# YuePanEdward/GH-ICP

Hardware: AMD Instinct MI355X
Metric: registered_pairs_per_sec (higher is better)
Workload: dtype f64

## Files before the change

gh-icp_amd/api.py:

```python
from __future__ import annotations

import ctypes as C
import os

import numpy as np

_HERE = os.path.dirname(os.path.abspath(__file__))
LIB_PATH = os.environ.get("GHICP_LIB") or os.path.join(_HERE, "libghicp_hip.so")

FEATURE_BSC, FEATURE_ROPS, FEATURE_FPFH, FEATURE_NONE = 0, 1, 2, 3
CORR_NN, CORR_NNR, CORR_KM = 0, 1, 2


class Params(C.Structure):
    _fields_ = [("feature", C.c_int32), ("corr", C.c_int32), ("dof", C.c_int32), ("max_iter", C.c_int32),
                ("radius_nonmax", C.c_float), ("adjust_ratio", C.c_float), ("adjust_step", C.c_float),
                ("est_iou", C.c_float), ("converge_t", C.c_float), ("converge_r", C.c_float),
                ("bbx_magnitude", C.c_float), ("pad_", C.c_float),
                ("penalty_initial", C.c_double), ("para1", C.c_double), ("para2", C.c_double),
                ("km_eps", C.c_double), ("min_cor", C.c_int32), ("weight_changing_rate", C.c_int32)]


class Iter(C.Structure):
    _fields_ = [("cor", C.c_int32), ("converged", C.c_int32)] + [
# ... 169 lines not shown
            raise GhicpError("ghicp error %d: %s" % (rc, self.lib.ghicp_last_error(self.h).decode()))

    def sync(self):
        self._check(self.lib.ghicp_ctx_synchronize(self.h))

    def kernel_timing(self, on=True):
        self._check(self.lib.ghicp_ctx_kernel_timing(self.h, 1 if on else 0))

    def km_launch_stats(self):
        out = (C.c_double * 8)()
        self._check(self.lib.ghicp_ctx_km_launch_stats(self.h, out))
        keys = ("launches", "solves", "mean_solve_ms", "mean_longest_solve_ms", "mean_launch_span_ms", "slots", "idle_slot_fraction", "worst_longest_over_mean")
        return dict(zip(keys, (float(v) for v in out)))

    def pair_loop_stats(self):
        out = (C.c_double * 8)()
        self._check(self.lib.ghicp_ctx_pair_loop_stats(self.h, out))
        keys = ("launches", "slots", "solves", "mean_solve_ms", "longest_solve_ms", "mean_launch_span_ms", "idle_slot_fraction", "solve_share_of_slot_time")
        return dict(zip(keys, (float(v) for v in out)))

    def loop_progress(self):
        a, t = C.c_int64(0), C.c_int64(0)
        self.lib.ghicp_ctx_loop_progress(self.h, C.byref(a), C.byref(t))
        return a.value, t.value

    def loop_progress_reset(self, total):
        self._check(self.lib.ghicp_ctx_loop_progress_reset(self.h, C.c_int64(int(total))))

    def set_loop_cost_hints(self, cost):
        c = np.ascontiguousarray(cost, dtype=np.float32)
        self._check(self.lib.ghicp_ctx_set_loop_cost_hints(self.h, C.c_int32(c.size), c.ctypes.data_as(C.POINTER(C.c_float))))

    def loop_timeline(self, detail=False):
# ... 501 lines not shown
```

gh-icp_amd/csrc/ctx.h:

```cpp
#pragma once
#include <hip/hip_runtime.h>

#include <atomic>
#include <cstdarg>
#include <cstdio>
#include <cstring>
#include <string>
#include <vector>

#include "../../include/ghicp_c.h"

#define GH_HIP(call)                                                                                          \
  do {                                                                                                        \
    hipError_t e_ = (call);                                                                                   \
    if (e_ != hipSuccess) return ctx->fail(GHICP_ERR_HIP, "%s:%d %s -> %s", __FILE__, __LINE__, #call, hipGetErrorString(e_)); \
  } while (0)
#define GH_TRY(call)               \
  do {                             \
    int r_ = (call);               \
    if (r_ != GHICP_OK) return r_; \
  } while (0)
#define GH_ARG(cond)                                                                \
  do {                                                                              \
    if (!(cond)) return ctx->fail(GHICP_ERR_ARG, "%s: bad argument (%s)", __func__, #cond); \
// ... 23 lines not shown
  }
  template <typename T> T* as() const { return reinterpret_cast<T*>(p); }
  void release() { if (p) (void)hipFree(p); p = nullptr; cap = 0; }
};

enum BufSlot {
  B_STAGE0 = 0, B_STAGE1, B_STAGE2, B_STAGE3, B_STAGE4, B_STAGE5, B_STAGE6, B_STAGE7,
  B_LOOP_STATE, B_LOOP_KPS, B_LOOP_PARTMIN, B_LOOP_PARTIDX, B_LOOP_PARTSUM, B_LOOP_PARTMIN2, B_LOOP_PARTIDX2, B_LOOP_FDT,
  B_LOOP_SP, B_LOOP_TP, B_LOOP_TRACE, B_LOOP_WFD, B_LOOP_KMW, B_LOOP_KMMATCH, B_LOOP_KMSCR, B_LOOP_ACC,
  B_GRID_KEYS, B_GRID_KEYS2, B_GRID_VALS, B_GRID_VALS2, B_GRID_TMP, B_GRID_START, B_GRID_PTS, B_GRID_MISC,
  B_GRID2_KEYS, B_GRID2_KEYS2, B_GRID2_VALS, B_GRID2_VALS2, B_GRID2_START, B_GRID2_PTS,
  B_FE_LAMBDA, B_FE_CURV, B_FE_COUNT, B_FE_CAND, B_FE_STATE, B_FE_KP, B_FE_SORTK, B_FE_SORTK2, B_FE_SORTV, B_FE_SORTV2, B_FE_CPTS,
  B_FE_FLAGS, B_FE_SCAN, B_FE_SCATTER,
  B_P_KEEP_S, B_P_KEEP_T, B_P_DS_S, B_P_DS_T, B_P_KP_S, B_P_KP_T, B_P_KPXYZ_S, B_P_KPXYZ_T, B_P_FEAT_S, B_P_FEAT_T, B_P_LCS,
  B_P_FD, B_P_MISC, B_P_PATTERN, B_FD_JOBS, B_TRANSFORM_JOBS,
  B_KM_LX, B_KM_MISC, B_KM_SLACK, B_KM_LSTAT, B_KM_ORDER,
  B_FB_DESC, B_FB_HEADPOS, B_FB_DS, B_FB_ORD,
  B_PRIM_TMP, B_NMSR_KEY, B_NMSR_CELL, B_NMSR_TABLE, B_NMSR_HEAD, B_NMSR_PTS, B_NMSR_SKEY, B_NMSR_STATE, B_NMSR_NEXT, B_NMSR_SEL, B_NMSR_MISC, B_NMSR_LIST, B_NMSR_PTS0, B_NMSR_SKEY0,
  B_ICP_TC_KEYS, B_ICP_TC_KEYS2, B_ICP_TC_VALS, B_ICP_TC_VALS2, B_ICP_TC_START, B_ICP_TC_PTS,
  B_ICP_SC_KEYS, B_ICP_SC_KEYS2, B_ICP_SC_VALS, B_ICP_SC_VALS2, B_ICP_SC_START, B_ICP_SC_PTS,
  B_ICP_CUR, B_ICP_Q, B_ICP_NN, B_ICP_ND, B_ICP_NN2, B_ICP_ND2, B_ICP_KEYS, B_ICP_KEYS2, B_ICP_SORTTMP, B_ICP_PART, B_ICP_STATE,
  B_ICP_PEND, B_ICP_TNRM, B_ICP_OUT,
  B_GICP_COVS, B_GICP_COVT, B_GICP_MAHAL, B_GICP_SRC4,
  B_NUM
};

enum KtSlot { KT_PCA = 0, KT_BSC, KT_KM_SOLVE, KT_CD_ROWMIN, KT_KM_WEIGHTS, KT_FD_BSC, KT_NMS_ROUND, KT_VOXEL_SORT,
              KT_FB_VOXEL, KT_FB_GRID, KT_FB_PRUNE, KT_FB_RANK, KT_FB_OUT,
              KT_PAIR_LOOP,
              KT_TRANSFORM,
              KT_PAIR_LOOP_DISPATCH,
// ... 27 lines not shown
    if (!kt_on || !a) return;
    hipEvent_t b = kt_event();
    (void)hipEventRecord(b, st);
    kt_pending.push_back({slot, a, b});
  }
  void kt_collect() {
    for (auto& p : kt_pending) {
      float ms = 0;
      if (hipEventElapsedTime(&ms, p.a, p.b) == hipSuccess) { kt_ms[p.slot] += ms; kt_count[p.slot]++; }
      kt_pool.push_back(p.a);
      kt_pool.push_back(p.b);
    }
    kt_pending.clear();
  }
  static constexpr int KM_LSTAT_MAX = 8192;
  static constexpr int KM_LSTAT_W = 8;
  long long km_launches = 0;
  std::vector<int> km_slots;
  long long loop_hazards = 0;
  std::vector<float> loop_cost_hints;
  std::vector<long long> loop_timeline;
  std::atomic<long long> loop_active{0}, loop_total{0};
  bool bbox_valid = false;
  const float* bbox_ptr = nullptr;
  long long bbox_n = 0;
  int bbox_stride = 0;
  float bbox_mm[6] = {0, 0, 0, 0, 0, 0};
  int device = 0;
  hipStream_t stream = nullptr;
  hipStream_t own_stream = nullptr;
  bool km_stats = false, km_force_hazard = false;
  int loop_slots_cap = 0;
  bool loop_confine = true;
  double loop_confine_margin = 1.15;
  hipStream_t confine_stream = nullptr, rest_stream = nullptr;
  int confine_cus = 0;
  struct ConfinePair { int cus; hipStream_t confined, rest; };
  std::vector<ConfinePair> confine_cache;
  bool km_compact = true;
  int km_compact_from = 0;
  int km_kflags() const { return (km_force_hazard ? 4 : 0) | (km_compact_from << 8); }
  int loop_min_lds = 0;
  std::vector<uint32_t> cu_mask;
  std::vector<hipStream_t> aux_streams;
  std::vector<hipEvent_t> aux_events;
  int* progress_host = nullptr;
  std::atomic<bool> progress_live{false};
  bool host_ptrs = false;
  struct Staged { const void* host; size_t bytes; uint64_t fp; void* dev; uint64_t tick; };
  std::vector<Staged> staged;
  size_t staged_bytes = 0;
  uint64_t stage_tick = 0;
  long long staged_hits = 0, staged_misses = 0;
  void stage_clear() {
    if (staged.empty()) return;
    (void)hipStreamSynchronize(stream);
// ... 180 lines not shown
```

gh-icp_amd/csrc/ctx.hip:

```cpp
#include "ctx.h"
#include "devmath.h"

extern "C" const char* ghicp_version(void) { return "ghicp-hip 0.1 (gfx950)"; }

extern "C" void ghicp_params_default(ghicp_params* p) {
  if (!p) return;
  memset(p, 0, sizeof(*p));
  p->feature = GHICP_FEATURE_BSC;
  p->corr = GHICP_CORR_KM;
  p->dof = 6;
  p->max_iter = 200;
  p->radius_nonmax = 1.5f;
  p->adjust_ratio = 1.1f;
  p->adjust_step = 0.1f;
  p->est_iou = 0.6f;
  p->converge_t = 0.02f;
  p->converge_r = 0.02f;
  p->bbx_magnitude = 0.f;
  p->penalty_initial = 2.0;
  p->para1 = 1.0;
  p->para2 = 1.0;
  p->km_eps = 0.01;
  p->min_cor = 10;
  p->weight_changing_rate = 6;
// ... 3 lines not shown
  if (!out) return GHICP_ERR_ARG;
  *out = nullptr;
  int count = 0;
  if (hipGetDeviceCount(&count) != hipSuccess || count <= 0 || device < 0 || device >= count) return GHICP_ERR_NO_GPU;
  if (hipSetDevice(device) != hipSuccess) return GHICP_ERR_NO_GPU;
  hipDeviceProp_t prop;
  if (hipGetDeviceProperties(&prop, device) != hipSuccess) return GHICP_ERR_NO_GPU;
  ghicp_ctx* c = new ghicp_ctx();
  c->device = device;
  c->num_cu = prop.multiProcessorCount > 0 ? prop.multiProcessorCount : 256;
  c->km_stats = getenv("GHICP_KM_STATS") != nullptr;
  c->km_force_hazard = getenv("GHICP_KM_FORCE_HAZARD") != nullptr;
  if (const char* e = getenv("GHICP_LOOP_SLOTS")) c->loop_slots_cap = atoi(e) > 0 ? atoi(e) : 0;
  if (const char* e = getenv("GHICP_LOOP_CONFINE")) c->loop_confine = atoi(e) != 0;
  if (const char* e = getenv("GHICP_KM_COMPACT")) c->km_compact = atoi(e) != 0;
  if (const char* e = getenv("GHICP_KM_COMPACT_FROM")) c->km_compact_from = atoi(e) > 0 && atoi(e) < 65535 ? atoi(e) : 0;
  if (const char* e = getenv("GHICP_LOOP_MIN_LDS")) c->loop_min_lds = atoi(e) > 0 ? atoi(e) : 0;
  if (const char* e = getenv("GHICP_LOOP_CONFINE_MARGIN")) { const double m = atof(e); if (m >= 0.25 && m <= 4.0) c->loop_confine_margin = m; }
  if (hipHostMalloc(&c->pinned, 4096, hipHostMallocDefault) != hipSuccess) { delete c; return GHICP_ERR_HIP; }
  c->pinned_cap = 4096;
  *out = c;
  return GHICP_OK;
}

extern "C" int ghicp_ctx_destroy(ghicp_ctx* ctx) {
  if (!ctx) return GHICP_OK;
  (void)hipSetDevice(ctx->device);
  (void)hipDeviceSynchronize();
  ctx->kt_collect();
  for (hipEvent_t e : ctx->kt_pool) (void)hipEventDestroy(e);
// ... 398 lines not shown
```

gh-icp_amd/csrc/km4.hip:

```cpp
#include "km4_dev.h"

#include <algorithm>
#include <vector>
#include <cstdlib>

namespace {

template <bool PROF, bool CP>
__global__ __launch_bounds__(K4_T, CP ? 4 : 1) void k_km4(const Km2Problem* __restrict__ probs, int flags, int lds_bytes, unsigned long long* __restrict__ lstat,
                                                        const int* __restrict__ order, unsigned short* __restrict__ scr, long long scr_stride) {
  const Km2Problem P = probs[order ? order[blockIdx.x] : (int)blockIdx.x];
  if (P.n <= 0 || (P.done && *P.done)) return;
  if (k4_takes_compact(P.n, flags, lds_bytes) != CP) return;
  extern __shared__ __attribute__((aligned(16))) char smem[];
  k4_solve_block<PROF, CP>(P, flags, smem, lds_bytes, lstat, CP && scr ? (k4_gu16)(scr + (size_t)blockIdx.x * (size_t)scr_stride) : (k4_gu16) nullptr);
}

}

size_t gh_km4_lds_bytes_compact(int n) { return (size_t)k4_lds_need(n, true) + 16; }

size_t gh_km4_slot_bytes(int n, bool compact_on) {
  const size_t quarter = 160 * 1024 / 4, std_b = gh_km4_lds_bytes(n);
  return (compact_on && std_b > quarter && gh_km4_lds_bytes_compact(n) <= quarter) ? gh_km4_lds_bytes_compact(n) : std_b;
// ... 129 lines not shown
    worst = std::max(worst, (double)r[3] / ((double)r[2] / (double)r[4]));
  }
  if (used == 0) return GHICP_OK;
  out8[0] = (double)used; out8[1] = solves; out8[2] = sum_dt / solves * tick_ms; out8[3] = sum_max / (double)used * tick_ms;
  out8[4] = sum_span / (double)used * tick_ms; out8[5] = slots; out8[6] = cap > 0 ? 1.0 - sum_dt / cap : 0.0; out8[7] = worst;
  return GHICP_OK;
}

extern "C" int ghicp_ctx_loop_hazards(ghicp_ctx* ctx, int64_t* solves) {
  GH_ENTER(ctx);
  GH_ARG(solves != nullptr);
  *solves = (int64_t)ctx->loop_hazards;
  return GHICP_OK;
}

extern "C" int ghicp_ctx_pair_loop_stats(ghicp_ctx* ctx, double* out8) {
  GH_ENTER(ctx);
  GH_ARG(out8 != nullptr);
  for (int i = 0; i < 8; i++) out8[i] = 0.0;
  const long long nl = ctx->km_launches;
  if (nl <= 0 || !ctx->buf[B_KM_LSTAT].p) return GHICP_OK;
  for (hipStream_t a : ctx->aux_streams) GH_HIP(hipStreamSynchronize(a));
  GH_HIP(hipStreamSynchronize(ctx->stream));
  constexpr int W = ghicp_ctx::KM_LSTAT_W;
  std::vector<unsigned long long> h((size_t)nl * W);
  GH_HIP(hipMemcpy(h.data(), ctx->buf[B_KM_LSTAT].p, h.size() * sizeof(unsigned long long), hipMemcpyDeviceToHost));
  const double tick_ms = 1e3 / 100e6;
  double launches = 0, slots = 0, solves = 0, sum_dt = 0, mx = 0, sum_span = 0, life = 0, cap = 0;
  for (long long l = 0; l < nl; l++) {
    const unsigned long long* r = &h[(size_t)l * W];
    if (r[6] == 0) continue;
    const double start = (double)((1ull << 62) - r[0]), span = (double)r[1] - start;
    launches++; slots += (double)r[6]; solves += (double)r[4]; sum_dt += (double)r[2]; mx = std::max(mx, (double)r[3]);
    sum_span += span; life += (double)r[5]; cap += std::min((double)ctx->km_slots[(size_t)l], (double)r[6]) * span;
  }
  if (launches == 0) return GHICP_OK;
  out8[0] = launches; out8[1] = slots; out8[2] = solves; out8[3] = solves > 0 ? sum_dt / solves * tick_ms : 0.0; out8[4] = mx * tick_ms;
  out8[5] = sum_span / launches * tick_ms; out8[6] = cap > 0 ? 1.0 - life / cap : 0.0; out8[7] = life > 0 ? sum_dt / life : 0.0;
  return GHICP_OK;
}
```

gh-icp_amd/csrc/loop.hip:

```cpp
#include "ctx.h"
#include "devmath.h"

#include <cmath>

#include "km_prob.h"
#include "km4_dev.h"
int gh_km_solve_dev(ghicp_ctx* ctx, const double* w, int n, double eps, int32_t* match, const int* done_flag);

namespace {

struct LoopState {
  int it, done, cor, converged_flag;
  double RMS, FDM, FDstd, IoU, para1, para2, penalty, CDmean, CDstd, energy;
  double Rt_till[16];
  double rmse_after;
  unsigned long long t_begin, t_end;
  unsigned long long t_solve_max;
  int it_solve_max;
  unsigned hw_id;
};

struct LoopConst {
  int ks, kt, n, feature, corr, max_iter, min_cor, nchunk_a, nchunk_b, chunk_a, chunk_b, nparts;
  float scale, est_iou, adjust_ratio, adjust_step;
// ... 79 lines not shown
    if (threadIdx.x == 0) {
      const size_t b = (size_t)by * cdiv_dev(ka, ROWS) + bx;
      P.psum[b * 2] = bs;
      P.psum[b * 2 + 1] = bs2;
    }
  }
}

template <int FT, bool COLS>
__global__ __launch_bounds__(ROWS) void k_cd_rowmin(const LoopProb* __restrict__ probs) {
  const LoopProb& P = probs[blockIdx.z];
  if (P.st->done) return;
  __shared__ double sB[CHUNK_MAX * 3];
  __shared__ double red[16];
  dev_cd_rowmin<FT, COLS>(P, (int)blockIdx.x, (int)blockIdx.y, sB, red);
}

__device__ inline void dev_penalty(const LoopProb& P, double* red) {
  LoopState* st = P.st;
  const LoopConst& C = P.C;
  double s = 0, s2 = 0;
  for (int i = threadIdx.x; i < C.nparts; i += blockDim.x) { s += P.psum[i * 2]; s2 += P.psum[i * 2 + 1]; }
  s = gh_block_sum(s, red);
  s2 = gh_block_sum(s2, red);
  if (threadIdx.x == 0) {
    const int it = st->it;
    const double cnt = (double)C.ks * (double)C.kt;
    double piv, wfd0 = 0, wed0 = 1;
    if (C.feature == GHICP_FEATURE_BSC) { wfd0 = P.wfd[it]; wed0 = 1.0 - wfd0; }
    const double inv_k0 = 1.0 / (double)(it + 1);
    if (C.feature == GHICP_FEATURE_BSC) piv = cd_pivot<GHICP_FEATURE_BSC>(P, wed0, wfd0, inv_k0);
    else if (C.feature == GHICP_FEATURE_FPFH) piv = cd_pivot<GHICP_FEATURE_FPFH>(P, wed0, wfd0, inv_k0);
    else piv = cd_pivot<GHICP_FEATURE_NONE>(P, wed0, wfd0, inv_k0);
    const double dm = s / (double)C.kt / (double)C.ks;
    const double mean = piv + dm;
    double var = s2 / cnt - dm * dm;
    if (var < 0) var = 0;
    const double sd = sqrt(var);
    double pen;
    if (C.feature == GHICP_FEATURE_NONE) {
      pen = fmax(mean, 1.0);
      st->CDstd = 0;
    } else if (C.feature == GHICP_FEATURE_BSC) {
      const double wfd = P.wfd[it], wed = 1.0 - wfd;
      if (it > 1) pen = st->RMS * st->para1 * (double)C.scale * wed + (st->FDM + st->para2 * st->FDstd) * wfd;
      else pen = mean - C.penalty_initial * sd;
      pen = fmax(pen, 5.0);
      st->CDstd = sd;
    } else {
      if (it > 1) pen = st->RMS * st->para1 * (double)C.scale * st->para2;
      else pen = mean / C.penalty_initial;
      st->CDstd = 0;
    }
    st->CDmean = mean;
    st->penalty = pen;
  }
}

__global__ __launch_bounds__(256) void k_penalty(const LoopProb* __restrict__ probs) {
  const LoopProb& P = probs[blockIdx.x];
  if (P.st->done) return;
  __shared__ double red[16];
  dev_penalty(P, red);
}

// ... 356 lines not shown
    }
  __syncthreads();
  dev_penalty(P, red);
  __syncthreads();
}
template <int FT>
__device__ __noinline__ void pl_graph(const LoopProb& P, int* ired) {
  const int rb4 = cdiv_dev(P.C.n, 4);
  for (int bx = 0; bx < rb4; bx++) dev_km_csr<FT, 0>(P, bx);
  __syncthreads();
  dev_km_scan_desc(P, ired);
  __syncthreads();
  for (int bx = 0; bx < rb4; bx++) dev_km_csr<FT, 1>(P, bx);
  __syncthreads();
}
template <bool PROF>
__device__ __noinline__ void pl_km(const Km2Problem* desc, int km_flags, char* smem, int lds_bytes) {
  const Km2Problem KP = *desc;
  k4_solve_block<PROF, false>(KP, km_flags, smem, lds_bytes, nullptr, (k4_gu16) nullptr);
  __syncthreads();
}
template <bool PROF>
__device__ __noinline__ void pl_km_compact(const Km2Problem* desc, int km_flags, char* smem, int lds_bytes, k4_gu16 scr) {
  const Km2Problem KP = *desc;
  k4_solve_block<PROF, true>(KP, km_flags, smem, lds_bytes, nullptr, scr);
  __syncthreads();
}
template <int FT>
__device__ __noinline__ void pl_solve(const LoopProb& P, double* red, int* ired, double* sh) {
  dev_solve<FT>(P, red, ired, sh);
  __syncthreads();
}

template <int FT, bool PROF>
__global__ __launch_bounds__(K4_T, 4) void k_pair_loop(const LoopProb* __restrict__ probs, const int* __restrict__ order, const int npairs, int* qhead,
                                                  const int km_flags, const int lds_bytes, unsigned long long* lstat, int* progress,
                                                  const int* __restrict__ order2, const int npairs2, int* qhead2,
                                                  unsigned short* __restrict__ scr, const long long scr_stride) {
  extern __shared__ __attribute__((aligned(16))) char smem[];
  double* sB = reinterpret_cast<double*>(smem);
  double* red = sB + CHUNK_MAX * 3;
  double* sh = red + 16;
  int* ired = reinterpret_cast<int*>(sh + 32);
  volatile int* s_idx = ired + 18;
  const unsigned long long t_slot0 = lstat ? __builtin_amdgcn_s_memrealtime() : 0ull;
  unsigned long long t_solve = 0ull, t_solve_max = 0ull, n_solve = 0ull;
  __builtin_amdgcn_s_setprio(3);
  for (int qsel = 0; qsel < 2; qsel++) {
  const int* const ord = qsel == 0 ? order : order2;
  const int np = qsel == 0 ? npairs : npairs2;
  int* const qh = qsel == 0 ? qhead : qhead2;
  if (ord == nullptr) break;
  for (;;) {
    __syncthreads();
    if (threadIdx.x == 0) *s_idx = atomicAdd(qh, 1);
    __syncthreads();
    const int q = *s_idx;
    if (q >= np) break;
    const LoopProb& P = probs[ord[q]];
    if (threadIdx.x == 0 && lstat) P.st->t_begin = __builtin_amdgcn_s_memrealtime();
    unsigned long long t_pair_max = 0ull;
    int it_pair_max = 0;
    while (*(volatile int*)&P.st->done == 0) {
      pl_sweep<FT>(P, sB, red);
      pl_graph<FT>(P, ired);
      const unsigned long long t0 = lstat ? __builtin_amdgcn_s_memrealtime() : 0ull;
      if (k4_takes_compact(P.C.n, km_flags, lds_bytes))
        pl_km_compact<PROF>(P.km_desc, km_flags, smem, lds_bytes, scr ? (k4_gu16)(scr + (size_t)blockIdx.x * (size_t)scr_stride) : (k4_gu16) nullptr);
      else
        pl_km<PROF>(P.km_desc, km_flags, smem, lds_bytes);
      if (lstat) {
        const unsigned long long dt = __builtin_amdgcn_s_memrealtime() - t0;
        t_solve += dt; t_solve_max = dt > t_solve_max ? dt : t_solve_max; n_solve++;
        if (dt > t_pair_max) { t_pair_max = dt; it_pair_max = *(volatile int*)&P.st->it; }
      }
      pl_solve<FT>(P, red, ired, sh);
    }
    if (threadIdx.x == 0 && lstat) {
      P.st->t_end = __builtin_amdgcn_s_memrealtime();
      P.st->t_solve_max = t_pair_max;
      P.st->it_solve_max = it_pair_max;
      P.st->hw_id = ((unsigned)__builtin_amdgcn_s_getreg((4) | (0 << 6) | (31 << 11)) & 0xFFFFu) | (((unsigned)__builtin_amdgcn_s_getreg((20) | (0 << 6) | (3 << 11)) & 0xFu) << 16);
    }
    if (threadIdx.x == 0 && progress) __hip_atomic_fetch_add(progress, 1, __ATOMIC_RELAXED, __HIP_MEMORY_SCOPE_SYSTEM);
  }
  }
  if (threadIdx.x == 0 && lstat) {
    const unsigned long long t1 = __builtin_amdgcn_s_memrealtime();
    atomicMax(&lstat[0], (1ull << 62) - t_slot0);
    atomicMax(&lstat[1], t1);
    atomicAdd(&lstat[2], t_solve);
    atomicMax(&lstat[3], t_solve_max);
    atomicAdd(&lstat[4], n_solve);
    atomicAdd(&lstat[5], t1 - t_slot0);
    atomicAdd(&lstat[6], 1ull);
  }
}

static void pick_chunks(int ka, int kb, int batch, int* chunk, int* nchunk) {
  const int rowblocks = cdiv(ka > 0 ? ka : 1, ROWS) * (batch > 0 ? batch : 1);
  int want = cdiv(2048, rowblocks);
  int ch = cdiv(kb > 0 ? kb : 1, want);
  if (ch < 32) ch = 32;
  if (ch > CHUNK_MAX) ch = CHUNK_MAX;
  *chunk = ch;
  *nchunk = kb > 0 ? cdiv(kb, ch) : 1;
}

struct Carver {
  char* base;
// ... 49 lines not shown
  size_t scr_next = 0;
  {
    int n_all = 1;
    bool need = ctx->km_compact_from > 0;
    for (int c = 0; c < nc; c++) {
      n_all = std::max(n_all, plan.nmax[c]);
      const size_t lds = std::max(std::max(plan.lds[c], (size_t)PL_SCRATCH + 64), (size_t)ctx->loop_min_lds);
      need = need || k4_lds_need(plan.nmax[c], false) > (long long)lds;
    }
    if (need) {
      scr_stride = k4_scratch_u16(n_all);
      size_t slots = 0;
      for (int c = 0; c < nc; c++) slots += 2 * (size_t)std::min(plan.count[c], 4 * ctx->num_cu);
      GH_TRY(ctx->reserve(B_KM_SLACK, slots * (size_t)scr_stride, &scr));
    }
  }
  GH_HIP(hipMemsetAsync(dqheads, 0, 16 * sizeof(int), s));
  unsigned long long* lstat = nullptr;
  int batch_slots = 0, batch_grid = 0;
  if (ctx->kt_on && ctx->km_launches < ghicp_ctx::KM_LSTAT_MAX) {
    GH_TRY(ctx->reserve(B_KM_LSTAT, (size_t)ghicp_ctx::KM_LSTAT_MAX * ghicp_ctx::KM_LSTAT_W, &lstat));
    lstat += ctx->km_launches * ghicp_ctx::KM_LSTAT_W;
  }
  int confine_b = 0;
  if (ctx->loop_confine && nc == 2 && plan.per_cu[0] == 3 && plan.per_cu[1] == 4 && plan.count[0] > 0 && plan.count[1] > 0 && ctx->cu_mask.empty() &&
      ctx->num_cu >= 8 && ctx->num_cu <= 2048 && plan.weight[0] > 0 && plan.weight[1] > 0) {
    const double w = std::min(0.9, ctx->loop_confine_margin * plan.weight[0] / (plan.weight[0] + plan.weight[1]));
    int B = (int)std::ceil(w * 4.0 * ctx->num_cu / (3.0 + w));
    B = std::max(B, (plan.count[0] >= 3 ? 1 : 0));
    B = std::min(B, std::min(ctx->num_cu / 2, cdiv(plan.count[0], 3)));
// ... 44 lines not shown
    GH_HIP_JOIN(hipOccupancyMaxActiveBlocksPerMultiprocessor(&per_cu, fn, K4_T, lds));
    if (per_cu <= 0) gh_join_aux(ctx);
    if (per_cu <= 0) return ctx->fail(GHICP_ERR_INTERNAL, "pair loop: a workgroup with %zu bytes of LDS does not fit a CU", lds);
    const int slots = per_cu * (confined ? (c == 0 ? confine_b : ctx->num_cu - confine_b) : ctx->num_cu);
    int grid = std::min(plan.count[c], slots);
    if (ctx->loop_slots_cap > 0) grid = std::min(grid, ctx->loop_slots_cap);
    batch_slots = std::max(batch_slots, per_cu * ctx->num_cu);
    batch_grid += grid;
    hipEvent_t kd = ctx->kt_begin_on(KT_PAIR_LOOP_DISPATCH, sc);
    const bool steal = confined && c == 0 && plan.lds[1] <= lds;
    stole = stole || steal;
    const int* o2 = steal ? (const int*)(plan.d_order + plan.begin[1]) : (const int*)nullptr;
    const int n2 = steal ? plan.count[1] : 0;
    int* q2 = steal ? dqheads + 1 : (int*)nullptr;
    unsigned short* scr_c = scr ? scr + scr_next * (size_t)scr_stride : nullptr;
    scr_next += (size_t)grid;
    if (prof)
      hipLaunchKernelGGL((k_pair_loop<FT, true>), dim3(grid), dim3(K4_T), lds, sc, dprobs, (const int*)(plan.d_order + plan.begin[c]), plan.count[c],
                         dqheads + c, kflags, (int)lds, lstat, ctx->progress_host, o2, n2, q2, scr_c, scr_stride);
    else
      hipLaunchKernelGGL((k_pair_loop<FT, false>), dim3(grid), dim3(K4_T), lds, sc, dprobs, (const int*)(plan.d_order + plan.begin[c]), plan.count[c],
                         dqheads + c, kflags, (int)lds, lstat, ctx->progress_host, o2, n2, q2, scr_c, scr_stride);
    ctx->kt_end_on(KT_PAIR_LOOP_DISPATCH, kd, sc);
    GH_HIP_JOIN(hipGetLastError());
    if (c > 0 || confined) {
      GH_HIP_JOIN(hipEventRecord(ctx->aux_events[(size_t)c + 1], sc));
      GH_HIP_JOIN(hipStreamWaitEvent(s, ctx->aux_events[(size_t)c + 1], 0));
    }
    if (confined && c == 1 && !stole) {
      const int grid2 = std::min(plan.count[c], per_cu * confine_b);
      unsigned short* scr_c2 = scr ? scr + scr_next * (size_t)scr_stride : nullptr;
      scr_next += (size_t)grid2;
      hipEvent_t kd2 = ctx->kt_begin_on(KT_PAIR_LOOP_DISPATCH, ctx->confine_stream);
      if (prof)
        hipLaunchKernelGGL((k_pair_loop<FT, true>), dim3(grid2), dim3(K4_T), lds, ctx->confine_stream, dprobs, (const int*)(plan.d_order + plan.begin[c]),
                           plan.count[c], dqheads + c, kflags, (int)lds, lstat, ctx->progress_host, (const int*)nullptr, 0, (int*)nullptr, scr_c2, scr_stride);
      else
        hipLaunchKernelGGL((k_pair_loop<FT, false>), dim3(grid2), dim3(K4_T), lds, ctx->confine_stream, dprobs, (const int*)(plan.d_order + plan.begin[c]),
                           plan.count[c], dqheads + c, kflags, (int)lds, lstat, ctx->progress_host, (const int*)nullptr, 0, (int*)nullptr, scr_c2, scr_stride);
      ctx->kt_end_on(KT_PAIR_LOOP_DISPATCH, kd2, ctx->confine_stream);
      GH_HIP_JOIN(hipGetLastError());
      batch_grid += grid2;
      GH_HIP_JOIN(hipEventRecord(ctx->aux_events[(size_t)nc + 1], ctx->confine_stream));
      GH_HIP_JOIN(hipStreamWaitEvent(s, ctx->aux_events[(size_t)nc + 1], 0));
    }
  }
  ctx->kt_end(KT_PAIR_LOOP, kt);
  if (lstat) {
    ctx->km_slots.push_back(std::min(batch_slots, batch_grid));
    ctx->km_launches++;
  }
  GH_HIP_JOIN(hipStreamSynchronize(s));
  return GHICP_OK;
}
// ... 361 lines not shown
```

include/ghicp_c.h:

```cpp
#ifndef GHICP_C_H_
#define GHICP_C_H_

#include <stddef.h>
#include <stdint.h>

#ifdef __cplusplus
extern "C" {
#endif

typedef struct ghicp_ctx ghicp_ctx;

enum {
  GHICP_OK = 0,
  GHICP_ERR_ARG = 1,
  GHICP_ERR_HIP = 2,
  GHICP_ERR_NO_GPU = 3,
  GHICP_ERR_CAPACITY = 4,
  GHICP_ERR_INTERNAL = 5
};

enum { GHICP_FEATURE_BSC = 0, GHICP_FEATURE_ROPS = 1, GHICP_FEATURE_FPFH = 2, GHICP_FEATURE_NONE = 3 };
enum { GHICP_CORR_NN = 0, GHICP_CORR_NNR = 1, GHICP_CORR_KM = 2 };

typedef struct ghicp_params {
// ... 15 lines not shown
  double Rt[16];
} ghicp_iter;

int ghicp_ctx_create(int device, ghicp_ctx** ctx);
int ghicp_ctx_destroy(ghicp_ctx* ctx);
int ghicp_ctx_set_stream(ghicp_ctx* ctx, void* hip_stream);
int ghicp_ctx_set_cu_mask(ghicp_ctx* ctx, const uint32_t* mask, int32_t n_words);
int ghicp_ctx_set_host_pointers(ghicp_ctx* ctx, int on);
int ghicp_ctx_stage_stats(const ghicp_ctx* ctx, int64_t* hits, int64_t* misses, int64_t* bytes_kept);
int ghicp_ctx_stage_clear(ghicp_ctx* ctx);
int ghicp_ctx_synchronize(ghicp_ctx* ctx);
const char* ghicp_last_error(const ghicp_ctx* ctx);
int ghicp_ctx_kernel_timing(ghicp_ctx* ctx, int on);
int ghicp_ctx_kernel_time(ghicp_ctx* ctx, const char* name, double* total_ms, int64_t* launches);
int ghicp_ctx_km_launch_stats(ghicp_ctx* ctx, double* out8);
int ghicp_ctx_pair_loop_stats(ghicp_ctx* ctx, double* out8);
int ghicp_ctx_loop_hazards(ghicp_ctx* ctx, int64_t* solves );
int ghicp_ctx_set_loop_cost_hints(ghicp_ctx* ctx, int32_t n_pairs, const float* cost);
int ghicp_ctx_loop_timeline(ghicp_ctx* ctx, int64_t* out3, int64_t cap_pairs, int64_t* n_pairs);
int ghicp_ctx_loop_progress(const ghicp_ctx* ctx, int64_t* active, int64_t* total);
int ghicp_ctx_loop_progress_reset(ghicp_ctx* ctx, int64_t total);
const char* ghicp_version(void);
void ghicp_params_default(ghicp_params* p);

int ghicp_voxel_filter(ghicp_ctx* ctx, const float* xyz, int64_t n, int stride, float voxel, int32_t* keep_idx, int64_t* m);
int ghicp_sort_pairs(ghicp_ctx* ctx, int key_bytes, const void* keys_in, void* keys_out, const uint32_t* vals_in, uint32_t* vals_out, int64_t n,
                     int bit_begin, int bit_end);
int ghicp_scan_inclusive_u32(ghicp_ctx* ctx, uint32_t* data, int64_t n);
int ghicp_select_flagged(ghicp_ctx* ctx, const uint8_t* flags, const uint32_t* vals, int64_t n, uint32_t* out, int64_t* count);
int ghicp_unique_sorted_u32(ghicp_ctx* ctx, const uint32_t* keys, int64_t n, uint32_t* out, int64_t* count);
int ghicp_gather_points(ghicp_ctx* ctx, const float* xyz, int stride, const int32_t* idx, int64_t m, float* out_xyz4);
// ... 188 lines not shown
```

Measured before the change: 411.8.

## Fuse KM candidate-mask construction into the cost sweep of the pair loop

Adds a fused path in the persistent pair-loop kernel. From iteration two on, the combined-distance sweep also evaluates the (predictable) penalty threshold and writes a per-row candidate bitmask, counts and row maxima. The graph build then fills the CSR from that mask instead of recomputing all distances, and a wave-ballot mask builder covers the first iterations. Target keypoints are cached in LDS when they fit, and per-stage timing counters are added. It costs a per-slot mask buffer and more code in the persistent kernel, which may raise register or LDS pressure.

```diff
diff --git a/gh-icp_amd/api.py b/gh-icp_amd/api.py
--- a/gh-icp_amd/api.py
+++ b/gh-icp_amd/api.py
@@ -207,9 +207,10 @@
         return dict(zip(keys, (float(v) for v in out)))
 
     def pair_loop_stats(self):
-        out = (C.c_double * 8)()
+        out = (C.c_double * 12)()
         self._check(self.lib.ghicp_ctx_pair_loop_stats(self.h, out))
-        keys = ("launches", "slots", "solves", "mean_solve_ms", "longest_solve_ms", "mean_launch_span_ms", "idle_slot_fraction", "solve_share_of_slot_time")
+        keys = ("launches", "slots", "solves", "mean_solve_ms", "longest_solve_ms", "mean_launch_span_ms", "idle_slot_fraction", "solve_share_of_slot_time",
+                "sweep_ms_per_iteration", "graph_ms_per_iteration", "tail_ms_per_iteration")
         return dict(zip(keys, (float(v) for v in out)))
 
     def loop_progress(self):
diff --git a/gh-icp_amd/csrc/ctx.h b/gh-icp_amd/csrc/ctx.h
--- a/gh-icp_amd/csrc/ctx.h
+++ b/gh-icp_amd/csrc/ctx.h
@@ -61,7 +61,7 @@
   B_FE_FLAGS, B_FE_SCAN, B_FE_SCATTER,
   B_P_KEEP_S, B_P_KEEP_T, B_P_DS_S, B_P_DS_T, B_P_KP_S, B_P_KP_T, B_P_KPXYZ_S, B_P_KPXYZ_T, B_P_FEAT_S, B_P_FEAT_T, B_P_LCS,
   B_P_FD, B_P_MISC, B_P_PATTERN, B_FD_JOBS, B_TRANSFORM_JOBS,
-  B_KM_LX, B_KM_MISC, B_KM_SLACK, B_KM_LSTAT, B_KM_ORDER,
+  B_KM_LX, B_KM_MISC, B_KM_SLACK, B_KM_LSTAT, B_KM_ORDER, B_KM_MASK,
   B_FB_DESC, B_FB_HEADPOS, B_FB_DS, B_FB_ORD,
   B_PRIM_TMP, B_NMSR_KEY, B_NMSR_CELL, B_NMSR_TABLE, B_NMSR_HEAD, B_NMSR_PTS, B_NMSR_SKEY, B_NMSR_STATE, B_NMSR_NEXT, B_NMSR_SEL, B_NMSR_MISC, B_NMSR_LIST, B_NMSR_PTS0, B_NMSR_SKEY0,
   B_ICP_TC_KEYS, B_ICP_TC_KEYS2, B_ICP_TC_VALS, B_ICP_TC_VALS2, B_ICP_TC_START, B_ICP_TC_PTS,
@@ -119,7 +119,7 @@
     kt_pending.clear();
   }
   static constexpr int KM_LSTAT_MAX = 8192;
-  static constexpr int KM_LSTAT_W = 8;
+  static constexpr int KM_LSTAT_W = 12;
   long long km_launches = 0;
   std::vector<int> km_slots;
   long long loop_hazards = 0;
@@ -145,6 +145,7 @@
   bool km_compact = true;
   int km_compact_from = 0;
   int km_kflags() const { return (km_force_hazard ? 4 : 0) | (km_compact_from << 8); }
+  bool loop_fuse = true;
   int loop_min_lds = 0;
   std::vector<uint32_t> cu_mask;
   std::vector<hipStream_t> aux_streams;
diff --git a/gh-icp_amd/csrc/ctx.hip b/gh-icp_amd/csrc/ctx.hip
--- a/gh-icp_amd/csrc/ctx.hip
+++ b/gh-icp_amd/csrc/ctx.hip
@@ -41,6 +41,7 @@
   if (const char* e = getenv("GHICP_LOOP_SLOTS")) c->loop_slots_cap = atoi(e) > 0 ? atoi(e) : 0;
   if (const char* e = getenv("GHICP_LOOP_CONFINE")) c->loop_confine = atoi(e) != 0;
   if (const char* e = getenv("GHICP_KM_COMPACT")) c->km_compact = atoi(e) != 0;
+  if (const char* e = getenv("GHICP_LOOP_FUSE")) c->loop_fuse = atoi(e) != 0;
   if (const char* e = getenv("GHICP_KM_COMPACT_FROM")) c->km_compact_from = atoi(e) > 0 && atoi(e) < 65535 ? atoi(e) : 0;
   if (const char* e = getenv("GHICP_LOOP_MIN_LDS")) c->loop_min_lds = atoi(e) > 0 ? atoi(e) : 0;
   if (const char* e = getenv("GHICP_LOOP_CONFINE_MARGIN")) { const double m = atof(e); if (m >= 0.25 && m <= 4.0) c->loop_confine_margin = m; }
diff --git a/gh-icp_amd/csrc/km4.hip b/gh-icp_amd/csrc/km4.hip
--- a/gh-icp_amd/csrc/km4.hip
+++ b/gh-icp_amd/csrc/km4.hip
@@ -167,10 +167,11 @@
   return GHICP_OK;
 }
 
-extern "C" int ghicp_ctx_pair_loop_stats(ghicp_ctx* ctx, double* out8) {
+extern "C" int ghicp_ctx_pair_loop_stats(ghicp_ctx* ctx, double* out12) {
   GH_ENTER(ctx);
-  GH_ARG(out8 != nullptr);
-  for (int i = 0; i < 8; i++) out8[i] = 0.0;
+  GH_ARG(out12 != nullptr);
+  double* const out8 = out12;
+  for (int i = 0; i < 12; i++) out12[i] = 0.0;
   const long long nl = ctx->km_launches;
   if (nl <= 0 || !ctx->buf[B_KM_LSTAT].p) return GHICP_OK;
   for (hipStream_t a : ctx->aux_streams) GH_HIP(hipStreamSynchronize(a));
@@ -179,16 +180,18 @@
   std::vector<unsigned long long> h((size_t)nl * W);
   GH_HIP(hipMemcpy(h.data(), ctx->buf[B_KM_LSTAT].p, h.size() * sizeof(unsigned long long), hipMemcpyDeviceToHost));
   const double tick_ms = 1e3 / 100e6;
-  double launches = 0, slots = 0, solves = 0, sum_dt = 0, mx = 0, sum_span = 0, life = 0, cap = 0;
+  double launches = 0, slots = 0, solves = 0, sum_dt = 0, mx = 0, sum_span = 0, life = 0, cap = 0, stage[3] = {0, 0, 0};
   for (long long l = 0; l < nl; l++) {
     const unsigned long long* r = &h[(size_t)l * W];
     if (r[6] == 0) continue;
     const double start = (double)((1ull << 62) - r[0]), span = (double)r[1] - start;
     launches++; slots += (double)r[6]; solves += (double)r[4]; sum_dt += (double)r[2]; mx = std::max(mx, (double)r[3]);
     sum_span += span; life += (double)r[5]; cap += std::min((double)ctx->km_slots[(size_t)l], (double)r[6]) * span;
+    for (int k = 0; k < 3; k++) stage[k] += (double)r[8 + k];
   }
   if (launches == 0) return GHICP_OK;
   out8[0] = launches; out8[1] = slots; out8[2] = solves; out8[3] = solves > 0 ? sum_dt / solves * tick_ms : 0.0; out8[4] = mx * tick_ms;
   out8[5] = sum_span / launches * tick_ms; out8[6] = cap > 0 ? 1.0 - life / cap : 0.0; out8[7] = life > 0 ? sum_dt / life : 0.0;
+  for (int k = 0; k < 3; k++) out12[8 + k] = solves > 0 ? stage[k] / solves * tick_ms : 0.0;
   return GHICP_OK;
 }
diff --git a/gh-icp_amd/csrc/loop.hip b/gh-icp_amd/csrc/loop.hip
--- a/gh-icp_amd/csrc/loop.hip
+++ b/gh-icp_amd/csrc/loop.hip
@@ -117,6 +117,14 @@
   __shared__ double sB[CHUNK_MAX * 3];
   __shared__ double red[16];
   dev_cd_rowmin<FT, COLS>(P, (int)blockIdx.x, (int)blockIdx.y, sB, red);
+}
+
+__device__ inline double gh_penalty_from_state(const LoopState* st, const LoopConst& C, const double* wfdtab, const int it) {
+  if (C.feature == GHICP_FEATURE_BSC) {
+    const double wfd = wfdtab[it], wed = 1.0 - wfd;
+    return fmax(st->RMS * st->para1 * (double)C.scale * wed + (st->FDM + st->para2 * st->FDstd) * wfd, 5.0);
+  }
+  return st->RMS * st->para1 * (double)C.scale * st->para2;
 }
 
 __device__ inline void dev_penalty(const LoopProb& P, double* red) {
@@ -145,13 +153,11 @@
       pen = fmax(mean, 1.0);
       st->CDstd = 0;
     } else if (C.feature == GHICP_FEATURE_BSC) {
-      const double wfd = P.wfd[it], wed = 1.0 - wfd;
-      if (it > 1) pen = st->RMS * st->para1 * (double)C.scale * wed + (st->FDM + st->para2 * st->FDstd) * wfd;
-      else pen = mean - C.penalty_initial * sd;
-      pen = fmax(pen, 5.0);
+      if (it > 1) pen = gh_penalty_from_state(st, C, P.wfd, it);
+      else pen = fmax(mean - C.penalty_initial * sd, 5.0);
       st->CDstd = sd;
     } else {
-      if (it > 1) pen = st->RMS * st->para1 * (double)C.scale * st->para2;
+      if (it > 1) pen = gh_penalty_from_state(st, C, P.wfd, it);
       else pen = mean / C.penalty_initial;
       st->CDstd = 0;
     }
@@ -538,6 +544,199 @@
   for (int bx = 0; bx < rb4; bx++) dev_km_csr<FT, 1>(P, bx);
   __syncthreads();
 }
+constexpr int PL_KPT_OFF = (PL_SCRATCH + 15) & ~15;
+
+template <int FT, typename V>
+__device__ inline double combined_distance_v(double ed, V f, double wed, double wfd, double inv_k) {
+  if (FT == GHICP_FEATURE_BSC) return wed * ed + wfd * (double)f;
+  if (FT == GHICP_FEATURE_FPFH) return 1.0 * ed / pow((double)f, inv_k);
+  return ed;
+}
+template <int FT> struct FdType { typedef uint16_t T; };
+template <> struct FdType<GHICP_FEATURE_FPFH> { typedef float T; };
+
+template <int FT, bool MEMB>
+__device__ __noinline__ void pl_sweep_km(const LoopProb& P, double* sB, double* red, double* sT, unsigned* mask) {
+  typedef typename FdType<FT>::T fd_t;
+  const LoopConst& C = P.C;
+  const int ks = C.ks, kt = C.kt, chunk = C.chunk_b, nchunk = C.nchunk_b;
+  const int rbA = cdiv_dev(ks > 0 ? ks : 1, ROWS);
+  const int it = P.st->it;
+  const fd_t* F = reinterpret_cast<const fd_t*>(P.FDt);
+  double wfd = 0, wed = 1;
+  if (FT == GHICP_FEATURE_BSC) { wfd = P.wfd[it]; wed = 1.0 - wfd; }
+  const double inv_k = 1.0 / (double)(it + 1);
+  const double dscale = (double)C.scale;
+  const double piv = cd_pivot<FT>(P, wed, wfd, inv_k);
+  const double pen = MEMB ? gh_penalty_from_state(P.st, C, P.wfd, it) : 0.0;
+  const int nw32 = 2 * cdiv_dev(kt, 64);
+  if (sT) {
+    __syncthreads();
+    for (int t = threadIdx.x; t < kt * 3; t += ROWS) sT[t] = P.kpT[t];
+    __syncthreads();
+  }
+  for (int by = 0; by < nchunk; by++) {
+    const int jb = by * chunk;
+    const int je = min(kt, jb + chunk);
+    if (sT == nullptr) {
+      __syncthreads();
+      for (int t = threadIdx.x; t < (je - jb) * 3; t += ROWS) sB[t] = P.kpT[(size_t)jb * 3 + t];
+      __syncthreads();
+    }
+    const double* tB = sT ? sT + (size_t)jb * 3 : sB;
+    const int jw = (MEMB && by == nchunk - 1) ? nw32 * 32 : je;
+    for (int bx = 0; bx < rbA; bx++) {
+      const int a = bx * ROWS + threadIdx.x;
+      double s = 0, s2 = 0;
+      if (a < ks) {
+        const double ax = P.kpS[(size_t)a * 3], ay = P.kpS[(size_t)a * 3 + 1], az = P.kpS[(size_t)a * 3 + 2];
+        unsigned cnt = 0;
+        double mx = -pen;
+        if (MEMB && by > 0) { cnt = P.km_cnt[a]; mx = P.km_lx[a]; }
+        for (int j0 = jb; j0 < jw; j0 += 32) {
+          unsigned bits = 0;
+          if (j0 + 32 <= je) {
+            for (int u0 = 0; u0 < 32; u0 += 4) {
+              fd_t f[4];
+              if (FT != GHICP_FEATURE_NONE) {
+#pragma unroll
+                for (int k = 0; k < 4; k++) f[k] = F[(size_t)(j0 + u0 + k) * ks + a];
+              }
+#pragma unroll
+              for (int k = 0; k < 4; k++) {
+                const int jj = j0 + u0 + k - jb;
+                const double dx = ax - tB[jj * 3], dy = ay - tB[jj * 3 + 1], dz = az - tB[jj * 3 + 2];
+                const double ed = dscale * sqrt(dx * dx + dy * dy + dz * dz);
+                const double cd = combined_distance_v<FT>(ed, FT != GHICP_FEATURE_NONE ? f[k] : (fd_t)0, wed, wfd, inv_k);
+                const double c0 = cd - piv;
+                s += c0;
+                s2 += c0 * c0;
+                if (MEMB && cd < pen) { bits |= 1u << (u0 + k); cnt++; mx = fmax(mx, -cd); }
+              }
+            }
+          } else {
+            for (int j = j0; j < je; j++) {
+              const int jj = j - jb;
+              const double dx = ax - tB[jj * 3], dy = ay - tB[jj * 3 + 1], dz = az - tB[jj * 3 + 2];
+              const double ed = dscale * sqrt(dx * dx + dy * dy + dz * dz);
+              const double cd = combined_distance_v<FT>(ed, FT != GHICP_FEATURE_NONE ? F[(size_t)j * ks + a] : (fd_t)0, wed, wfd, inv_k);
+              const double c0 = cd - piv;
+              s += c0;
+              s2 += c0 * c0;
+              if (MEMB && cd < pen) { bits |= 1u << (j - j0); cnt++; mx = fmax(mx, -cd); }
+            }
+          }
+          if (MEMB) mask[(size_t)(j0 >> 5) * ks + a] = bits;
+        }
+        if (MEMB) { P.km_cnt[a] = cnt; P.km_lx[a] = mx; }
+      }
+      const double bs = gh_block_sum(s, red);
+      const double bs2 = gh_block_sum(s2, red);
+      if (threadIdx.x == 0) {
+        const size_t b = (size_t)by * rbA + bx;
+        P.psum[b * 2] = bs;
+        P.psum[b * 2 + 1] = bs2;
+      }
+    }
+  }
+  if (MEMB)
+    for (int i = ks + threadIdx.x; i < C.n; i += ROWS) { P.km_cnt[i] = 0u; P.km_lx[i] = -pen; }
+  __syncthreads();
+  dev_penalty(P, red);
+  __syncthreads();
+}
+
+template <int FT>
+__device__ inline void dev_km_count_mask(const LoopProb& P, const double* sT, unsigned* mask) {
+  typedef typename FdType<FT>::T fd_t;
+  const LoopConst& C = P.C;
+  const int wave = threadIdx.x >> 6, lane = threadIdx.x & 63;
+  const double pen = P.st->penalty;
+  const int it = P.st->it;
+  double wfd = 0, wed = 1;
+  if (FT == GHICP_FEATURE_BSC) { wfd = P.wfd[it]; wed = 1.0 - wfd; }
+  const double inv_k = 1.0 / (double)(it + 1);
+  const double* tB = sT ? sT : P.kpT;
+  const fd_t* F = reinterpret_cast<const fd_t*>(P.FD);
+  for (int i = wave; i < C.n; i += 4) {
+    if (i >= C.ks) {
+      if (lane == 0) { P.km_cnt[i] = 0u; P.km_lx[i] = -pen; }
+      continue;
+    }
+    const double sx = P.kpS[(size_t)i * 3], sy = P.kpS[(size_t)i * 3 + 1], sz = P.kpS[(size_t)i * 3 + 2];
+    unsigned c = 0;
+    double mx = -pen;
+    for (int j0 = 0; j0 < C.kt; j0 += 64) {
+      const int j = j0 + lane;
+      bool e = false;
+      if (j < C.kt) {
+        const double dx = sx - tB[(size_t)j * 3], dy = sy - tB[(size_t)j * 3 + 1], dz = sz - tB[(size_t)j * 3 + 2];
+        const double ed = (double)C.scale * sqrt(dx * dx + dy * dy + dz * dz);
+        const double cd = combined_distance_v<FT>(ed, FT != GHICP_FEATURE_NONE ? F[(size_t)i * C.kt + j] : (fd_t)0, wed, wfd, inv_k);
+        e = cd < pen;
+        if (e) mx = fmax(mx, -cd);
+      }
+      const unsigned long long b = __ballot(e);
+      if (lane == 0) {
+        mask[(size_t)(j0 >> 5) * C.ks + i] = (unsigned)b;
+        mask[(size_t)((j0 >> 5) + 1) * C.ks + i] = (unsigned)(b >> 32);
+      }
+      c += __popcll(b);
+    }
+    for (int o = 32; o > 0; o >>= 1) mx = fmax(mx, __shfl_xor(mx, o, 64));
+    if (lane == 0) { P.km_cnt[i] = c; P.km_lx[i] = mx; }
+  }
+}
+
+template <int FT>
+__device__ inline void dev_km_fill_mask(const LoopProb& P, const double* sT, const unsigned* mask) {
+  typedef typename FdType<FT>::T fd_t;
+  const LoopConst& C = P.C;
+  const int wave = threadIdx.x >> 6, lane = threadIdx.x & 63;
+  const int it = P.st->it;
+  double wfd = 0, wed = 1;
+  if (FT == GHICP_FEATURE_BSC) { wfd = P.wfd[it]; wed = 1.0 - wfd; }
+  const double inv_k = 1.0 / (double)(it + 1);
+  const double* tB = sT ? sT : P.kpT;
+  const fd_t* F = reinterpret_cast<const fd_t*>(P.FD);
+  int* __restrict__ cols = P.km_cols;
+  double* __restrict__ vals = P.km_vals;
+  const int nw = cdiv_dev(C.kt, 64);
+  const unsigned long long below = (1ull << lane) - 1ull;
+  for (int i = wave; i < C.ks; i += 4) {
+    const double sx = P.kpS[(size_t)i * 3], sy = P.kpS[(size_t)i * 3 + 1], sz = P.kpS[(size_t)i * 3 + 2];
+    const unsigned base = P.km_rptr[i], end = P.km_rptr[i + 1];
+    unsigned c = 0;
+    bool bad = false;
+    unsigned long long b = (unsigned long long)mask[i] | ((unsigned long long)mask[(size_t)C.ks + i] << 32);
+    for (int w = 0; w < nw; w++) {
+      const unsigned long long cur = b;
+      if (w + 1 < nw) b = (unsigned long long)mask[(size_t)(2 * w + 2) * C.ks + i] | ((unsigned long long)mask[(size_t)(2 * w + 3) * C.ks + i] << 32);
+      if (cur == 0ull) continue;
+      const int j = w * 64 + lane;
+      if ((cur >> lane) & 1ull) {
+        const double dx = sx - tB[(size_t)j * 3], dy = sy - tB[(size_t)j * 3 + 1], dz = sz - tB[(size_t)j * 3 + 2];
+        const double ed = (double)C.scale * sqrt(dx * dx + dy * dy + dz * dz);
+        const double cd = combined_distance_v<FT>(ed, FT != GHICP_FEATURE_NONE ? F[(size_t)i * C.kt + j] : (fd_t)0, wed, wfd, inv_k);
+        const unsigned off = base + c + __popcll(cur & below);
+        if (off < end) { cols[off] = j; vals[off] = -cd; }
+        else bad = true;
+      }
+      c += __popcll(cur);
+    }
+    if (bad || c != end - base) atomicOr(P.km_status, 0x100);
+  }
+}
+
+template <int FT, bool MEMB>
+__device__ __noinline__ void pl_graph_km(const LoopProb& P, int* ired, const double* sT, unsigned* mask) {
+  if (!MEMB) dev_km_count_mask<FT>(P, sT, mask);
+  __syncthreads();
+  dev_km_scan_desc(P, ired);
+  __syncthreads();
+  dev_km_fill_mask<FT>(P, sT, mask);
+  __syncthreads();
+}
 template <bool PROF>
 __device__ __noinline__ void pl_km(const Km2Problem* desc, int km_flags, char* smem, int lds_bytes) {
   const Km2Problem KP = *desc;
@@ -560,7 +759,8 @@
 __global__ __launch_bounds__(K4_T, 4) void k_pair_loop(const LoopProb* __restrict__ probs, const int* __restrict__ order, const int npairs, int* qhead,
                                                   const int km_flags, const int lds_bytes, unsigned long long* lstat, int* progress,
                                                   const int* __restrict__ order2, const int npairs2, int* qhead2,
-                                                  unsigned short* __restrict__ scr, const long long scr_stride) {
+                                                  unsigned short* __restrict__ scr, const long long scr_stride,
+                                                  unsigned* mask_all, const long long mask_stride) {
   extern __shared__ __attribute__((aligned(16))) char smem[];
   double* sB = reinterpret_cast<double*>(smem);
   double* red = sB + CHUNK_MAX * 3;
@@ -568,7 +768,7 @@
   int* ired = reinterpret_cast<int*>(sh + 32);
   volatile int* s_idx = ired + 18;
   const unsigned long long t_slot0 = lstat ? __builtin_amdgcn_s_memrealtime() : 0ull;
-  unsigned long long t_solve = 0ull, t_solve_max = 0ull, n_solve = 0ull;
+  unsigned long long t_solve = 0ull, t_solve_max = 0ull, n_solve = 0ull, t_sweep = 0ull, t_graph = 0ull, t_tail = 0ull;
   __builtin_amdgcn_s_setprio(3);
   for (int qsel = 0; qsel < 2; qsel++) {
   const int* const ord = qsel == 0 ? order : order2;
@@ -586,8 +786,23 @@
     unsigned long long t_pair_max = 0ull;
     int it_pair_max = 0;
     while (*(volatile int*)&P.st->done == 0) {
-      pl_sweep<FT>(P, sB, red);
-      pl_graph<FT>(P, ired);
+      unsigned* const mask = mask_all ? mask_all + (size_t)blockIdx.x * (size_t)mask_stride : (unsigned*)nullptr;
+      const bool fuse = mask != nullptr && (P.C.nchunk_b == 1 || (P.C.chunk_b & 31) == 0);
+      double* const sT = PL_KPT_OFF + (long long)P.C.kt * 24 <= (long long)lds_bytes ? reinterpret_cast<double*>(smem + PL_KPT_OFF) : (double*)nullptr;
+      if (lstat) t_sweep -= __builtin_amdgcn_s_memrealtime();
+      if (!fuse) {
+        pl_sweep<FT>(P, sB, red);
+        if (lstat) { const unsigned long long x = __builtin_amdgcn_s_memrealtime(); t_sweep += x; t_graph -= x; }
+        pl_graph<FT>(P, ired);
+      } else if (FT != GHICP_FEATURE_NONE && *(volatile int*)&P.st->it > 1) {
+        pl_sweep_km<FT, FT != GHICP_FEATURE_NONE>(P, sB, red, sT, mask);
+        if (lstat) { const unsigned long long x = __builtin_amdgcn_s_memrealtime(); t_sweep += x; t_graph -= x; }
+        pl_graph_km<FT, FT != GHICP_FEATURE_NONE>(P, ired, sT, mask);
+      } else {
+        pl_sweep_km<FT, false>(P, sB, red, sT, mask);
+        if (lstat) { const unsigned long long x = __builtin_amdgcn_s_memrealtime(); t_sweep += x; t_graph -= x; }
+        pl_graph_km<FT, false>(P, ired, sT, mask);
+      }
       const unsigned long long t0 = lstat ? __builtin_amdgcn_s_memrealtime() : 0ull;
       if (k4_takes_compact(P.C.n, km_flags, lds_bytes))
         pl_km_compact<PROF>(P.km_desc, km_flags, smem, lds_bytes, scr ? (k4_gu16)(scr + (size_t)blockIdx.x * (size_t)scr_stride) : (k4_gu16) nullptr);
@@ -595,10 +810,12 @@
         pl_km<PROF>(P.km_desc, km_flags, smem, lds_bytes);
       if (lstat) {
         const unsigned long long dt = __builtin_amdgcn_s_memrealtime() - t0;
+        t_graph += t0; t_tail -= t0 + dt;
         t_solve += dt; t_solve_max = dt > t_solve_max ? dt : t_solve_max; n_solve++;
         if (dt > t_pair_max) { t_pair_max = dt; it_pair_max = *(volatile int*)&P.st->it; }
       }
       pl_solve<FT>(P, red, ired, sh);
+      if (lstat) t_tail += __builtin_amdgcn_s_memrealtime();
     }
     if (threadIdx.x == 0 && lstat) {
       P.st->t_end = __builtin_amdgcn_s_memrealtime();
@@ -618,6 +835,9 @@
     atomicAdd(&lstat[4], n_solve);
     atomicAdd(&lstat[5], t1 - t_slot0);
     atomicAdd(&lstat[6], 1ull);
+    atomicAdd(&lstat[8], t_sweep);
+    atomicAdd(&lstat[9], t_graph);
+    atomicAdd(&lstat[10], t_tail);
   }
 }
 
@@ -697,6 +917,16 @@
       for (int c = 0; c < nc; c++) slots += 2 * (size_t)std::min(plan.count[c], 4 * ctx->num_cu);
       GH_TRY(ctx->reserve(B_KM_SLACK, slots * (size_t)scr_stride, &scr));
     }
+  }
+  unsigned* msk = nullptr;
+  long long msk_stride = 0;
+  if (ctx->loop_fuse) {
+    int n_all = 1;
+    for (int c = 0; c < nc; c++) n_all = std::max(n_all, plan.nmax[c]);
+    msk_stride = 2ll * cdiv(n_all, 64) * n_all;
+    size_t slots = 0;
+    for (int c = 0; c < nc; c++) slots += 2 * (size_t)std::min(plan.count[c], 4 * ctx->num_cu);
+    GH_TRY(ctx->reserve(B_KM_MASK, slots * (size_t)msk_stride, &msk));
   }
   GH_HIP(hipMemsetAsync(dqheads, 0, 16 * sizeof(int), s));
   unsigned long long* lstat = nullptr;
@@ -771,13 +1001,14 @@
     const int n2 = steal ? plan.count[1] : 0;
     int* q2 = steal ? dqheads + 1 : (int*)nullptr;
     unsigned short* scr_c = scr ? scr + scr_next * (size_t)scr_stride : nullptr;
+    unsigned* msk_c = msk ? msk + scr_next * (size_t)msk_stride : nullptr;
     scr_next += (size_t)grid;
     if (prof)
       hipLaunchKernelGGL((k_pair_loop<FT, true>), dim3(grid), dim3(K4_T), lds, sc, dprobs, (const int*)(plan.d_order + plan.begin[c]), plan.count[c],
-                         dqheads + c, kflags, (int)lds, lstat, ctx->progress_host, o2, n2, q2, scr_c, scr_stride);
+                         dqheads + c, kflags, (int)lds, lstat, ctx->progress_host, o2, n2, q2, scr_c, scr_stride, msk_c, msk_stride);
     else
       hipLaunchKernelGGL((k_pair_loop<FT, false>), dim3(grid), dim3(K4_T), lds, sc, dprobs, (const int*)(plan.d_order + plan.begin[c]), plan.count[c],
-                         dqheads + c, kflags, (int)lds, lstat, ctx->progress_host, o2, n2, q2, scr_c, scr_stride);
+                         dqheads + c, kflags, (int)lds, lstat, ctx->progress_host, o2, n2, q2, scr_c, scr_stride, msk_c, msk_stride);
     ctx->kt_end_on(KT_PAIR_LOOP_DISPATCH, kd, sc);
     GH_HIP_JOIN(hipGetLastError());
     if (c > 0 || confined) {
@@ -787,14 +1018,15 @@
     if (confined && c == 1 && !stole) {
       const int grid2 = std::min(plan.count[c], per_cu * confine_b);
       unsigned short* scr_c2 = scr ? scr + scr_next * (size_t)scr_stride : nullptr;
+      unsigned* msk_c2 = msk ? msk + scr_next * (size_t)msk_stride : nullptr;
       scr_next += (size_t)grid2;
       hipEvent_t kd2 = ctx->kt_begin_on(KT_PAIR_LOOP_DISPATCH, ctx->confine_stream);
       if (prof)
         hipLaunchKernelGGL((k_pair_loop<FT, true>), dim3(grid2), dim3(K4_T), lds, ctx->confine_stream, dprobs, (const int*)(plan.d_order + plan.begin[c]),
-                           plan.count[c], dqheads + c, kflags, (int)lds, lstat, ctx->progress_host, (const int*)nullptr, 0, (int*)nullptr, scr_c2, scr_stride);
+                           plan.count[c], dqheads + c, kflags, (int)lds, lstat, ctx->progress_host, (const int*)nullptr, 0, (int*)nullptr, scr_c2, scr_stride, msk_c2, msk_stride);
       else
         hipLaunchKernelGGL((k_pair_loop<FT, false>), dim3(grid2), dim3(K4_T), lds, ctx->confine_stream, dprobs, (const int*)(plan.d_order + plan.begin[c]),
-                           plan.count[c], dqheads + c, kflags, (int)lds, lstat, ctx->progress_host, (const int*)nullptr, 0, (int*)nullptr, scr_c2, scr_stride);
+                           plan.count[c], dqheads + c, kflags, (int)lds, lstat, ctx->progress_host, (const int*)nullptr, 0, (int*)nullptr, scr_c2, scr_stride, msk_c2, msk_stride);
       ctx->kt_end_on(KT_PAIR_LOOP_DISPATCH, kd2, ctx->confine_stream);
       GH_HIP_JOIN(hipGetLastError());
       batch_grid += grid2;
diff --git a/include/ghicp_c.h b/include/ghicp_c.h
--- a/include/ghicp_c.h
+++ b/include/ghicp_c.h
@@ -53,7 +53,7 @@
 int ghicp_ctx_kernel_timing(ghicp_ctx* ctx, int on);
 int ghicp_ctx_kernel_time(ghicp_ctx* ctx, const char* name, double* total_ms, int64_t* launches);
 int ghicp_ctx_km_launch_stats(ghicp_ctx* ctx, double* out8);
-int ghicp_ctx_pair_loop_stats(ghicp_ctx* ctx, double* out8);
+int ghicp_ctx_pair_loop_stats(ghicp_ctx* ctx, double* out12);
 int ghicp_ctx_loop_hazards(ghicp_ctx* ctx, int64_t* solves );
 int ghicp_ctx_set_loop_cost_hints(ghicp_ctx* ctx, int32_t n_pairs, const float* cost);
 int ghicp_ctx_loop_timeline(ghicp_ctx* ctx, int64_t* out3, int64_t cap_pairs, int64_t* n_pairs);
```

Result: faster. 423.5, median of 6 (+2.8%).
